# John-Jumper/Upside-MD

Measured on AMD Instinct MI355X. Metric: MD steps/sec (force evals/sec) per 300-res protein, higher is better.
Workload: dtype f32; 1 GPU; syn300_10A: 300-res synthetic protein, full side-chain BP, 10 A pair list (BASELINE.json configs[2]); 4096 independent replicas per GPU, T=0.8, dt=0.009, Langevin thermostat every round; replicas_per_gpu=4096, n_atom=900, settle_steps=100

## Files before the change

upside-md_amd/csrc/kernels_batch_impl.h:

```cpp
#pragma once
template <bool PAIR>
__global__ void __launch_bounds__(1024) PG_KERNEL_ATTR k_batch(BatchArgs A) {
    extern __shared__ __attribute__((aligned(16))) float lds[];
    const int w = blockIdx.x;
    int i = 0;
    while (i + 1 < A.n && w >= A.e[i].wg_end) ++i;
    const BatchEntryHdr& h = A.e[i];
    const int local = w - (i ? A.e[i - 1].wg_end : 0);
    const BX B = {local % h.gx, h.gx, local / h.gx, h.gy};
    const unsigned char* arg = A.blob + h.off;
    if constexpr (!PAIR) {
        const upk_igraph_t& G = *(const upk_igraph_t*)arg;
        const upk_rotamer_t& R = *(const upk_rotamer_t*)arg;
        switch (h.kind) {
            case BK_CHECK: d_pairlist_check(G, B, lds); break;
            case BK_BUILD_ROT: d_pairlist_build<true, UPK_IT_ROTAMER>(G, h.i0, h.i1, B, lds); break;
            case BK_BUILD_COV: d_pairlist_build<true, UPK_IT_HBOND_COVERAGE>(G, h.i0, h.i1, B, lds); break;
            case BK_BUILD_ENV: d_pairlist_build<true, UPK_IT_ENVIRONMENT>(G, h.i0, h.i1, B, lds); break;
            case BK_BUILD_HB: d_pairlist_build<true, UPK_IT_PROTEIN_HBOND>(G, h.i0, h.i1, B, lds); break;
            case BK_REFINE: d_pairlist_refine<false, unsigned short>(G, h.i0, h.i1, B, lds); break;
            case BK_REFINE_SYM: d_pairlist_refine<true, int>(G, h.i0, h.i1, B, lds); break;
            case BK_REFINE_SHORT: d_pairlist_refine_short(G, h.i0, B, lds); break;
            case BK_ORDER: d_pairlist_order(G, h.i0, B, lds); break;
            case BK_CLEAR_SLOTS: d_rotamer_clear_slots(R, B, lds); break;
            case BK_BUILD_SLOTS: d_rotamer_build_slots(R, B, lds); break;
            case BK_NBR_SLOTS: d_rotamer_nbr_slots(R, B, lds); break;
            case BK_SLOTS_BOTH: {
                d_rotamer_build_slots(R, B, lds);
                __syncthreads();
                const BX B1 = {0, 1, B.by, B.gy};
                d_rotamer_nbr_slots(R, B1, lds);
            } break;
            default: break;
        }
    } else {
        const upk_igraph_t& G = *(const upk_igraph_t*)arg;
        const PairArgs& P = *(const PairArgs*)(arg + ((sizeof(upk_igraph_t) + 15) & ~(size_t)15));
        switch (h.kind) {
            case BK_ROWS_HB_FWD: d_pair_rows<UPK_IT_PROTEIN_HBOND, 3, 0, false>(G, P, B, lds); break;
            case BK_ROWS_HB_BWD: d_pair_rows<UPK_IT_PROTEIN_HBOND, 3, 2, false>(G, P, B, lds); break;
            case BK_ROWS_ENV_FWD: d_pair_rows<UPK_IT_ENVIRONMENT, 1, 0, false>(G, P, B, lds); break;
            case BK_COV_ROWS2: d_cov_rows2<2, false>(G, P, B, lds); break;
            case BK_COV_ROWS2_POLY: d_cov_rows2<2, true>(G, P, B, lds); break;
            case BK_ENV_BWD: d_pair_backward<UPK_IT_ENVIRONMENT, 1, false>(G, P, B, lds); break;
            case BK_COV_BWD2: d_cov_backward2<2, false>(G, P, B, lds); break;
            case BK_COV_BWD2_POLY: d_cov_backward2<2, true>(G, P, B, lds); break;
            case BK_BWD_FINISH: d_pair_backward_finish(G, h.i0, h.d0, B, lds); break;
            default: break;
        }
    }
}

extern "C" void* upk_batch_create() { return new BatchState; }
extern "C" void upk_batch_destroy(void* b) {
    BatchState* s = (BatchState*)b;
    if (s && env_set("UPSIDE_HIP_FUSE_STATS")) fprintf(stderr, "merged launches: %ld launches for %ld kernels\n", s->n_merged, s->n_items);
    delete s;
}
extern "C" int upk_batch_begin(const upk_launch_t* L) {
    BatchState* s = batch_of(L);
    if (!s) return 0;
    UPK_FLUSH(L);
    s->open = true; s->chain = 0; s->chains.clear(); s->chain_fused.clear(); s->skip_nbr_slots = false;
    return 0;
}
extern "C" void upk_batch_chain(const upk_launch_t* L, int chain) { BatchState* s = batch_of(L); if (s) s->chain = chain; }
extern "C" int upk_batch_run(const upk_launch_t* L) {
    BatchState* s = batch_of(L);
    if (!s || !s->open) return 0;
    size_t n_stage = 0;
    for (auto& c : s->chains) n_stage = c.size() > n_stage ? c.size() : n_stage;
    for (size_t st = 0; st < n_stage; ++st) {
        for (int pair = 0; pair < 2; ++pair) {
            BatchArgs A; memset(&A, 0, sizeof(A));
            size_t used = 0, lds = 0; int wg = 0;
            auto launch = [&]() {
                if (!A.n) return;
                if (lds < 64) lds = 64;
                if (pair) hipLaunchKernelGGL(k_batch<true>, dim3(wg), dim3(1024), lds, ST(L), A);
                else hipLaunchKernelGGL(k_batch<false>, dim3(wg), dim3(1024), lds, ST(L), A);
                s->n_merged += 1; s->n_items += A.n;
                memset(&A, 0, sizeof(A)); used = 0; lds = 0; wg = 0;
            };
            for (auto& c : s->chains) {
                if (st >= c.size() || (int)bk_is_pair(c[st].kind) != pair) continue;
                const BatchItem& it = c[st];
                const size_t need = (it.args.size() + 15) & ~(size_t)15;
                if (A.n == BATCH_MAX_ENTRIES || used + need > BATCH_BLOB) launch();
                BatchEntryHdr& h = A.e[A.n++];
                h.kind = it.kind; h.gx = it.gx; h.gy = it.gy; h.i0 = it.i0; h.i1 = it.i1; h.d0 = it.d0; h.off = (int)used;
                memcpy(A.blob + used, it.args.data(), it.args.size()); used += need;
                wg += it.gx * it.gy; h.wg_end = wg;
                if (it.lds > lds) lds = it.lds;
            }
            launch();
        }
    }
    s->chains.clear();
    return launch_status();
}
extern "C" int upk_batch_end(const upk_launch_t* L) {
    BatchState* s = batch_of(L);
    if (!s || !s->open) return 0;
    const int r = upk_batch_run(L);
    s->open = false;
    return r;
}
```

upside-md_amd/csrc/kernels_igraph.hip:

```cpp
#include "igraph_device.h"
#include <cstring>

using namespace up;

#define ST(L) ((hipStream_t)(L)->stream)
#define ROWS_PER_BLOCK 4
#define IG_BLOCK (ROWS_PER_BLOCK * UP_WAVE)
#ifndef UPK_LAUNCH_STATUS_DEFINED
#define UPK_LAUNCH_STATUS_DEFINED
static inline int launch_status() { return (int)hipGetLastError(); }
#endif
static inline unsigned rows_grid(int n_rows) { return n_rows > 0 ? (unsigned)((n_rows + ROWS_PER_BLOCK - 1) / ROWS_PER_BLOCK) : 1u; }

#define C_OUT(c, s)  ((c).out  + (size_t)(s) * (c).n_elem * (c).stride)
#define C_SENS(c, s) ((c).sens + (size_t)(s) * (c).n_elem * (c).stride)


__device__ __forceinline__ float quadspline(const upk_igraph_t& G, const float* __restrict__ p, const float* x1, const float* x2,
                                            float* d1, float* d2) {
    const int ka = G.n_knot_angular, k = G.n_knot;
    const float inv_dx = G.inv_dx, inv_dtheta = G.inv_dtheta;
    const f3 displace = mk3(x2[0] - x1[0], x2[1] - x1[1], x2[2] - x1[2]);
    const f3 rvec1 = mk3(x1[3], x1[4], x1[5]), rvec2 = mk3(x2[3], x2[4], x2[5]);
    const float dist2 = mag2(displace), inv_dist = rsqrt_(dist2);
    const float dist_coord = dist2 * (inv_dist * inv_dx);
    const f3 u = inv_dist * displace;
    const float cos1 = dot(rvec1, u), cos2 = -dot(rvec2, u);
    float a1, da1, a2, da2, wide, dwide, narrow, dnarrow;
    deBoor_vd(a1, da1, p, (cos1 + 1.f) * inv_dtheta + 1.f);
    deBoor_vd(a2, da2, p + ka, (cos2 + 1.f) * inv_dtheta + 1.f);
    clamped_deBoor_vd(wide, dwide, p + 2 * ka, dist_coord, k);
    clamped_deBoor_vd(narrow, dnarrow, p + 2 * ka + k, dist_coord, k);
    const float angular_weight = a1 * a2;
    const float radial_deriv = inv_dx * (dwide + angular_weight * dnarrow);
    const float angular_deriv1 = inv_dtheta * da1 * a2 * narrow;
    const float angular_deriv2 = inv_dtheta * a1 * da2 * narrow;
    const f3 rXX = angular_deriv1 * rvec1 - angular_deriv2 * rvec2;
    const f3 deriv_dir = inv_dist * (rXX - dot(u, rXX) * u);
    const f3 dd = radial_deriv * u + deriv_dir;
    d1[0] = -dd.x; d1[1] = -dd.y; d1[2] = -dd.z;
    d1[3] = angular_deriv1 * u.x; d1[4] = angular_deriv1 * u.y; d1[5] = angular_deriv1 * u.z;
    d2[0] = dd.x; d2[1] = dd.y; d2[2] = dd.z;
    d2[3] = -angular_deriv2 * u.x; d2[4] = -angular_deriv2 * u.y; d2[5] = -angular_deriv2 * u.z;
    return wide + angular_weight * narrow;
}

__device__ __forceinline__ float hbond_coverage_edge(const upk_igraph_t& G, const float* __restrict__ p, const float* x1,
                                                     const float* x2, float* d1, float* d2) {
    const float coverage = quadspline(G, p, x1, x2, d1, d2);
    const float one_m = 1.f - x1[6];
    const float prefactor = one_m * one_m;
#pragma unroll
    for (int c = 0; c < 6; ++c) { d1[c] *= prefactor; d2[c] *= prefactor; }
    d1[6] = -coverage * one_m * 2.f;
    return prefactor * coverage;
}

__device__ __forceinline__ float radial_edge(const float* __restrict__ p, const float* x1, const float* x2, float* d1, float* d2) {
    const float inv_dx = p[0];
    const f3 disp = mk3(x1[0] - x2[0], x1[1] - x2[1], x1[2] - x2[2]);
    const float dist2 = mag2(disp), inv_dist = rsqrt_(dist2 + 1e-7f);
    const float dist_coord = dist2 * (inv_dist * inv_dx);
    float v, dv;
    clamped_deBoor_vd(v, dv, p + 1, dist_coord, 16);
    const float k = inv_dist * inv_dx * dv;
    d1[0] = disp.x * k; d1[1] = disp.y * k; d1[2] = disp.z * k;
    d2[0] = -d1[0]; d2[1] = -d1[1]; d2[2] = -d1[2];
    return v;
}

__device__ __forceinline__ float pair_eval(const upk_igraph_t& G, const float* __restrict__ p, const float* x1, const float* x2,
                                           float* d1, float* d2) {
    switch (G.itype) {
        case UPK_IT_RADIAL: case UPK_IT_HBOND_SC_RADIAL: return radial_edge(p, x1, x2, d1, d2);
        case UPK_IT_HBOND_COVERAGE: return hbond_coverage_edge(G, p, x1, x2, d1, d2);
        case UPK_IT_ENVIRONMENT: return environment_edge(p, x1, x2, d1, d2);
        case UPK_IT_PROTEIN_HBOND: return protein_hbond_edge(p, x1, x2, d1, d2);
        default: return quadspline(G, p, x1, x2, d1, d2);
    }
}

__device__ __forceinline__ bool acceptable_id_pair(int itype, int id1, int id2) {
    switch (itype) {
        case UPK_IT_ROTAMER: return ((unsigned)id1 >> 4) != ((unsigned)id2 >> 4);
        case UPK_IT_HBOND_COVERAGE:
        case UPK_IT_RADIAL: case UPK_IT_HBOND_SC_RADIAL:
        case UPK_IT_ENVIRONMENT: return (2 < id1 - id2) || (2 < id2 - id1);
        default: return true;
    }
}

__device__ __forceinline__ void load_elem(float* x, const upk_coord_t& node, int s, int loc, int dim) {
    const float* p = C_OUT(node, s) + (size_t)loc * node.stride;
#pragma unroll
    for (int c = 0; c < 8; ++c) x[c] = (c < dim) ? p[c] : 0.f;
}

__device__ __forceinline__ void d_pairlist_check(const upk_igraph_t& G, const BX B, float* lds_unused) {
    __shared__ int moved;
    __shared__ float top[2][16];
    const int s = B.by;
    if (threadIdx.x == 0) moved = 0;
    __syncthreads();
    const int n_tot = G.symmetric ? G.n1 : G.n1 + G.n2;
    float d1 = 0.f, d2 = 0.f;
    for (int e = threadIdx.x; e < n_tot; e += blockDim.x) {
        const bool side1 = e < G.n1;
        const int i = side1 ? e : e - G.n1;
        const upk_coord_t& node = side1 ? G.node1 : G.node2;
        const float* x = C_OUT(node, s) + (size_t)(side1 ? G.loc1[i] : G.loc2[i]) * node.stride;
        const float* c = (side1 ? G.cache_pos1 + (size_t)s * G.n1 * 4 : G.cache_pos2 + (size_t)s * G.n2 * 4) + (size_t)i * 4;
        const float4 xv = *(const float4*)x, cv = *(const float4*)c;
        const float x0 = xv.x, x1 = xv.y, x2 = xv.z;
        const float dx = x0 - cv.x, dy = x1 - cv.y, dz = x2 - cv.z;
        const float dd = dx * dx + dy * dy + dz * dz;
        d2 = fmaxf(d2, fminf(d1, dd)); d1 = fmaxf(d1, dd);
        ((float4*)(side1 ? G.cur_pos1 + (size_t)s * G.n1 * 4 : G.cur_pos2 + (size_t)s * G.n2 * 4))[i] = make_float4(x0, x1, x2, 0.f);
    }
    {
#pragma unroll
        for (int off = 32; off > 0; off >>= 1) {
            const float o1 = __shfl_xor(d1, off, UP_WAVE), o2 = __shfl_xor(d2, off, UP_WAVE);
            const float n1 = fmaxf(d1, o1), n2 = fmaxf(fminf(d1, o1), fmaxf(d2, o2));
            d1 = n1; d2 = n2;
        }
        if ((threadIdx.x & 63) == 0) { top[0][threadIdx.x >> 6] = d1; top[1][threadIdx.x >> 6] = d2; }
        __syncthreads();
        if (threadIdx.x == 0) {
            float a = 0.f, b = 0.f;
            for (int w = 0; w < (int)(blockDim.x >> 6); ++w) {
                const float o1 = top[0][w], o2 = top[1][w];
                const float n1 = fmaxf(a, o1), n2 = fmaxf(fminf(a, o1), fmaxf(b, o2));
                a = n1; b = n2;
            }
            const float margin = G.cache_cutoff - G.cutoff;
            if (sqrtf(a) + sqrtf(b) > 0.999f * margin) moved = 1;
        }
    }
    __syncthreads();
    if (moved) {
        for (int e = threadIdx.x; e < n_tot; e += blockDim.x) {
            const bool side1 = e < G.n1;
            const int i = side1 ? e : e - G.n1;
            const upk_coord_t& node = side1 ? G.node1 : G.node2;
            const float* x = C_OUT(node, s) + (size_t)(side1 ? G.loc1[i] : G.loc2[i]) * node.stride;
            float4* c = (float4*)(side1 ? G.cache_pos1 + (size_t)s * G.n1 * 4 : G.cache_pos2 + (size_t)s * G.n2 * 4) + i;
            *c = make_float4(x[0], x[1], x[2], __int_as_float(side1 ? G.id1[i] : G.id2[i]));
        }
        if (G.mark_table) {
            uint4* m = (uint4*)(G.mark_table + (size_t)s * G.mark_stride);
            const int n16 = G.mark_stride / 16;
            for (int i = threadIdx.x; i < n16; i += blockDim.x) m[i] = make_uint4(0, 0, 0, 0);
        }
    }
    if (threadIdx.x == 0) {
        G.rebuild_flag[s] = moved;
        int* fl = UPK_FLAG_LIST(G);
        if (moved) fl[1 + atomicAdd(&fl[0], 1)] = s;
        if (s == 0) G.flagged[(size_t)(G.parity ^ 1) * G.flag_stride] = 0;
    }
}
__global__ void k_pairlist_check(upk_igraph_t G)  { d_pairlist_check(G, BX_REAL, nullptr); }
static inline int upkeep_block(int n_system, int large) { return n_system >= 2 * upk_device_cu_count() ? 256 : large; }
extern "C" int upk_pairlist_check(const upk_launch_t* L, const upk_igraph_t* G) {
    if (batch_add(L, BK_CHECK, 1, L->n_system, 0, G, sizeof(*G))) return 0;
    UPK_FLUSH(L);
    const int n_tot = G->symmetric ? G->n1 : G->n1 + G->n2;
    const int threads = upkeep_block(L->n_system, n_tot <= 256 ? 256 : (n_tot <= 512 ? 512 : 1024));
    hipLaunchKernelGGL(k_pairlist_check, dim3(1, L->n_system), dim3(threads), 0, ST(L), *G);
    return launch_status();
}

static inline int plb_rows(int n_system) { return n_system >= upk_device_cu_count() ? 128 : 64; }
template <int IT>
__device__ __forceinline__ bool plb_id_ok(int id_row_side1, int id_other_side2) {
    if (IT == UPK_IT_ROTAMER) return ((unsigned)(id_row_side1 ^ id_other_side2)) > 15u;
    if (IT == UPK_IT_HBOND_COVERAGE || IT == UPK_IT_ENVIRONMENT || IT == UPK_IT_RADIAL || IT == UPK_IT_HBOND_SC_RADIAL) { const int d = id_row_side1 - id_other_side2; return (d > 2) | (d < -2); }
    return true;
}
__device__ __forceinline__ int plb_node_of(const upk_igraph_t& G, int id) {
    const int nr = (id >> 4) & 15;
    return (id >> 8) + ((-(int)(nr == 6) & G.mark_start6) | (-(int)(nr == 3) & G.mark_start3));
}
template <bool STAGED, int IT>
__device__ __forceinline__ void d_pairlist_build(const upk_igraph_t& G, int blocks1, int rows_per_wg, const BX B, float* plb_lds) {
        float4* oth = (float4*)plb_lds;
    constexpr bool SYM = IT == UPK_IT_ROTAMER || IT == UPK_IT_RADIAL;
    constexpr bool UPPER = IT == UPK_IT_ROTAMER;
    const int* fl = UPK_FLAG_LIST(G);
    const int n_flagged = fl[0];
    const int lane = threadIdx.x & 63, wave = __builtin_amdgcn_readfirstlane(threadIdx.x >> 6), n_wave = blockDim.x >> 6;
    const bool side1 = (int)B.bx < blocks1;
    const int rb = side1 ? B.bx : B.bx - blocks1;
    const int n_my = side1 ? G.n1 : G.n2, n_other = side1 ? G.n2 : G.n1;
    const int n_pad = (n_other + 63) & ~63;
    const int cap = side1 ? G.cap1 : G.cap2;
    const float cut2 = G.cache_cutoff * G.cache_cutoff;
    for (int fi = B.by; fi < n_flagged; fi += B.gy) {
        const int s = fl[1 + fi];
        const float4* src = (const float4*)((side1 ? G.cache_pos2 : G.cache_pos1) + (size_t)s * n_other * 4);
        const float4* mine = (const float4*)((side1 ? G.cache_pos1 : G.cache_pos2) + (size_t)s * n_my * 4);
        if (STAGED) {
            __syncthreads();
            for (int j = threadIdx.x; j < n_pad; j += blockDim.x) oth[j] = j < n_other ? src[j] : make_float4(1e18f, 1e18f, 1e18f, 0.f);
            __syncthreads();
        }
        float4 x_next = make_float4(0.f, 0.f, 0.f, 0.f);
        { const int i0 = rb * rows_per_wg + wave; if (wave < rows_per_wg && i0 < n_my) x_next = mine[i0]; }
        for (int r = wave; r < rows_per_wg; r += n_wave) {
            const int i = rb * rows_per_wg + r;
            if (i >= n_my) break;
            const float4 x = x_next;
            { const int in = i + n_wave; if (r + n_wave < rows_per_wg && in < n_my) x_next = mine[in]; }
            const int my_id = __float_as_int(x.w);
            typedef typename list_word<IT>::type W;
            W* nbr = (side1 ? (W*)G.nbr1 + (size_t)s * G.n1 * G.cap1 : (W*)G.nbr2 + (size_t)s * G.n2 * G.cap2) + (size_t)i * cap;
            int count = 0;
            const int my_node = SYM ? plb_node_of(G, my_id) : 0;
            for (int j0 = UPPER ? ((i + 1) & ~63) : 0; j0 < n_pad; j0 += 64) {
                const int j = j0 + lane;
                float4 y;
                if (STAGED) y = oth[j];
                else y = j < n_other ? src[j] : make_float4(1e18f, 1e18f, 1e18f, 0.f);
                const float d2 = dist2_exact(x.x, x.y, x.z, y.x, y.y, y.z);
                const int oid = __float_as_int(y.w);
                bool hit = (d2 < cut2) & (side1 ? plb_id_ok<IT>(my_id, oid) : plb_id_ok<IT>(oid, my_id));
                if (UPPER) hit = hit & (j > i);
                else if (SYM) hit = hit & (j != i);
                const unsigned long long b = __ballot(hit);
                if (!b) continue;
                const int pos = count + __popcll(b & ((1ull << lane) - 1ull));
                if (hit & (pos < cap)) nbr[pos] = (W)j;
                count += __popcll(b);
                if (SYM && G.mark_table) {
                    const bool up = hit & (j > i);
                    const int key = up ? plb_node_of(G, oid) : -1;
                    const int key_prev = __builtin_amdgcn_update_dpp(-1, key, 0x138 , 0xf, 0xf, false);
                    if (up & (key_prev != key)) {
                        unsigned char* mt = G.mark_table + (size_t)s * G.mark_stride;
                        mt[my_node * G.mark_ld + key] = 1; mt[key * G.mark_ld + my_node] = 1;
                    }
                }
            }
            if (lane == 0) {
                (side1 ? G.cnt1 + (size_t)s * G.n1 : G.cnt2 + (size_t)s * G.n2)[i] = count < cap ? count : cap;
                if (count > cap) *G.error_flag = 1;
            }
        }
    }
}
template <bool STAGED, int IT>
__global__ void __launch_bounds__(1024) k_pairlist_build(upk_igraph_t G, int blocks1, int rows_per_wg)  {
    extern __shared__ __attribute__((aligned(16))) float lds_dyn_[];
    d_pairlist_build<STAGED, IT>(G, blocks1, rows_per_wg, BX_REAL, lds_dyn_);
}
template <int IT>
static void plb_launch(const upk_launch_t* L, const upk_igraph_t* G, dim3 grid, size_t lds, bool staged, int blocks1) {
    const int rows = plb_rows(L->n_system);
    if (staged) hipLaunchKernelGGL((k_pairlist_build<true, IT>), grid, dim3(upkeep_block(L->n_system, 1024)), lds, ST(L), *G, blocks1, rows);
    else hipLaunchKernelGGL((k_pairlist_build<false, IT>), grid, dim3(1024), 0, ST(L), *G, blocks1, rows);
}
extern "C" int upk_pairlist_build(const upk_launch_t* L, const upk_igraph_t* G) { return upk_pairlist_build_sides(L, G, 3); }
extern "C" int upk_pairlist_build_sides(const upk_launch_t* L, const upk_igraph_t* G, int sides) {
    if (!list_words_match(G)) return 9010;
    const int rows = plb_rows(L->n_system);
    const int blocks1 = (sides & 1) ? (G->n1 + rows - 1) / rows : 0;
    const int blocks2 = (G->symmetric || !(sides & 2)) ? 0 : (G->n2 + rows - 1) / rows;
    if (blocks1 + blocks2 == 0) return 0;
    const int n_max = G->n1 > G->n2 ? G->n1 : G->n2;
    const size_t lds = (size_t)((n_max + 63) & ~63) * 16;
    const dim3 grid(blocks1 + blocks2, UPK_FLAG_GRID(L->n_system));
    static const bool force_unstaged = env_int("UPSIDE_HIP_PLB_UNSTAGED", 0) != 0;
    const bool staged = lds <= 150 * 1024 && !force_unstaged;
    if (staged) {
        const int bk = G->itype == UPK_IT_ROTAMER ? BK_BUILD_ROT : G->itype == UPK_IT_HBOND_COVERAGE ? BK_BUILD_COV : G->itype == UPK_IT_ENVIRONMENT ? BK_BUILD_ENV
                     : G->itype == UPK_IT_PROTEIN_HBOND ? BK_BUILD_HB : 0;
        if (bk && batch_add(L, bk, (int)grid.x, (int)grid.y, lds, G, sizeof(*G), nullptr, 0, blocks1, rows)) return 0;
    }
    UPK_FLUSH(L);
    switch (G->itype) {
        case UPK_IT_ROTAMER: plb_launch<UPK_IT_ROTAMER>(L, G, grid, lds, staged, blocks1); break;
        case UPK_IT_HBOND_COVERAGE: plb_launch<UPK_IT_HBOND_COVERAGE>(L, G, grid, lds, staged, blocks1); break;
        case UPK_IT_ENVIRONMENT: plb_launch<UPK_IT_ENVIRONMENT>(L, G, grid, lds, staged, blocks1); break;
        case UPK_IT_RADIAL: plb_launch<UPK_IT_RADIAL>(L, G, grid, lds, staged, blocks1); break;
        case UPK_IT_HBOND_SC_RADIAL: plb_launch<UPK_IT_HBOND_SC_RADIAL>(L, G, grid, lds, staged, blocks1); break;
        default: plb_launch<UPK_IT_PROTEIN_HBOND>(L, G, grid, lds, staged, blocks1); break;
    }
    return launch_status();
}

#ifndef PLR_BLOCK
#define PLR_BLOCK 256
#endif
#ifndef PLR_ROWS
#define PLR_ROWS 256
#endif
#ifndef PLR_DEPTH
#define PLR_DEPTH 2
#endif
static_assert(PLR_ROWS <= 64 * (PLR_BLOCK / 64), "a wavefront of the refine keeps the positions and list lengths of its rows one per lane: at most 64 rows per wavefront");
typedef float plr_v2 __attribute__((ext_vector_type(2)));
__device__ __forceinline__ plr_v2 dist2_exact2(plr_v2 ax, plr_v2 ay, plr_v2 az, plr_v2 bx, plr_v2 by, plr_v2 bz) {
#pragma clang fp contract(off)
    const plr_v2 dx = ax - bx, dy = ay - by, dz = az - bz;
    const plr_v2 xx = dx * dx, yy = dy * dy, zz = dz * dz;
    const plr_v2 s = xx + yy;
    return s + zz;
}
template <bool SYM, typename W>
__device__ __forceinline__ void d_pairlist_refine(const upk_igraph_t& G, int side, int rows_per_wg, const BX B, float* plr_lds) {
        float4* oth = (float4*)plr_lds;
    const int s = B.by;
    const int lane = threadIdx.x & 63, wave = __builtin_amdgcn_readfirstlane(threadIdx.x >> 6), n_wave = blockDim.x >> 6;
    const bool rows1 = side == 1;
    const int n_rows = rows1 ? G.n1 : G.n2, n_other = rows1 ? G.n2 : G.n1;
    const int cap = rows1 ? G.cap1 : G.cap2;
    const float4* src = (const float4*)((rows1 ? G.cur_pos2 : G.cur_pos1) + (size_t)s * n_other * 4);
    const float4* mine = (const float4*)((rows1 ? G.cur_pos1 : G.cur_pos2) + (size_t)s * n_rows * 4);
    for (int j = threadIdx.x; j <= n_other; j += blockDim.x) oth[j] = j < n_other ? src[j] : make_float4(1e18f, 1e18f, 1e18f, 0.f);
    __syncthreads();
    const int dead = n_other;
    const W* nbr_base = (const W*)(rows1 ? G.nbr1 : G.nbr2) + (size_t)s * n_rows * cap;
    const int* cnt_arr = (rows1 ? G.cnt1 : G.cnt2) + (size_t)s * n_rows;
    W* hit_base = (W*)(rows1 ? G.hit1 : G.hit2) + (size_t)s * n_rows * cap;
    int* hcnt = (rows1 ? G.hcnt1 : G.hcnt2) + (size_t)s * n_rows;
    int* hlo = (SYM && G.hlo1) ? G.hlo1 + (size_t)s * n_rows : nullptr;
    const float cut2 = G.cutoff * G.cutoff;
    const int jmask = G.nbr_j_bits ? (1 << G.nbr_j_bits) - 1 : 0x7fffffff;
    const int per_wave = (rows_per_wg + n_wave - 1) / n_wave;
    const int r0 = B.bx * rows_per_wg + wave * per_wave;
    int r1 = r0 + per_wave; { const int wg_end = (B.bx + 1) * rows_per_wg; if (r1 > wg_end) r1 = wg_end; if (r1 > n_rows) r1 = n_rows; }
    if (r0 >= r1) return;
    const bool have = r0 + lane < r1;
    const float4 my_x = have ? mine[r0 + lane] : make_float4(0.f, 0.f, 0.f, 0.f);
    const int my_cnt = have ? cnt_arr[r0 + lane] : 0;
    int my_n = 0, my_lo = 0;
    auto bcast = [&](float v, int l) { return __int_as_float(__builtin_amdgcn_readlane(__float_as_int(v), l)); };
    auto fetch_pair = [&](int ra, int& a, int& b) {
        a = dead; b = dead;
        if (ra < r1) {
            const int la = ra - r0;
            const int cA = __builtin_amdgcn_readlane(my_cnt, la & 63), cB = ra + 1 < r1 ? __builtin_amdgcn_readlane(my_cnt, (la + 1) & 63) : 0;
            if (lane < cA) a = nbr_base[(size_t)ra * cap + lane];
            if (lane < cB) b = nbr_base[(size_t)(ra + 1) * cap + lane];
        }
    };
    int qA[PLR_DEPTH], qB[PLR_DEPTH];
#pragma unroll
    for (int d = 0; d < PLR_DEPTH; ++d) fetch_pair(r0 + 2 * d, qA[d], qB[d]);
    for (int ra = r0; ra < r1; ra += 2) {
        const int la = ra - r0, lb = la + 1;
        const bool hasB = ra + 1 < r1;
        const int cntA = __builtin_amdgcn_readlane(my_cnt, la), cntB = hasB ? __builtin_amdgcn_readlane(my_cnt, lb & 63) : 0;
        int wA = qA[0], wB = qB[0];
#pragma unroll
        for (int d = 0; d + 1 < PLR_DEPTH; ++d) { qA[d] = qA[d + 1]; qB[d] = qB[d + 1]; }
        fetch_pair(ra + 2 * PLR_DEPTH, qA[PLR_DEPTH - 1], qB[PLR_DEPTH - 1]);
        plr_v2 xx, xy, xz;
        xx.x = bcast(my_x.x, la); xy.x = bcast(my_x.y, la); xz.x = bcast(my_x.z, la);
        xx.y = bcast(my_x.x, lb & 63); xy.y = bcast(my_x.y, lb & 63); xz.y = bcast(my_x.z, lb & 63);
        const W* nbrA = nbr_base + (size_t)ra * cap; const W* nbrB = nbrA + cap;
        W* outA = hit_base + (size_t)ra * cap; W* outB = outA + cap;
        int na = 0, nb = 0, loa = 0, lob = 0;
        const int cmax = cntA > cntB ? cntA : cntB;
        for (int k0 = 0; k0 < cmax; k0 += 64) {
            const int k = k0 + lane;
            if (k0) { wA = k < cntA ? nbrA[k] : dead; wB = k < cntB ? nbrB[k] : dead; }
            const int jA = wA & jmask, jB = wB & jmask;
            const float4 yA = oth[jA], yB = oth[jB];
            plr_v2 yx, yy, yz; yx.x = yA.x; yx.y = yB.x; yy.x = yA.y; yy.y = yB.y; yz.x = yA.z; yz.y = yB.z;
            const plr_v2 d2 = dist2_exact2(xx, xy, xz, yx, yy, yz);
            const bool hitA = d2.x < cut2, hitB = d2.y < cut2;
            const unsigned long long mA = __builtin_amdgcn_ballot_w64(hitA), mB = __builtin_amdgcn_ballot_w64(hitB);
            const unsigned long long below = (1ull << lane) - 1ull;
            if (hitA) outA[na + __popcll(mA & below)] = (W)wA;
            if (hitB) outB[nb + __popcll(mB & below)] = (W)wB;
            na += __popcll(mA); nb += __popcll(mB);
            if (SYM) { loa += __popcll(__builtin_amdgcn_ballot_w64(hitA && jA < ra)); lob += __popcll(__builtin_amdgcn_ballot_w64(hitB && jB < ra + 1)); }
        }
        if (lane == la) { my_n = na; my_lo = loa; }
        if (hasB && lane == lb) { my_n = nb; my_lo = lob; }
    }
    if (have) { hcnt[r0 + lane] = my_n; if (SYM && hlo) hlo[r0 + lane] = my_lo; }
}
template <bool SYM, typename W>
__global__ void __launch_bounds__(PLR_BLOCK) k_pairlist_refine(upk_igraph_t G, int side, int rows_per_wg)  {
    extern __shared__ __attribute__((aligned(16))) float lds_dyn_[];
    d_pairlist_refine<SYM, W>(G, side, rows_per_wg, BX_REAL, lds_dyn_);
}
__device__ __forceinline__ void d_pairlist_refine_short(const upk_igraph_t& G, int side, const BX B, float* lds_unused) {
    const int s = B.by, row = B.bx * blockDim.x + threadIdx.x;
    const bool rows1 = side == 1;
    const int n_rows = rows1 ? G.n1 : G.n2, n_other = rows1 ? G.n2 : G.n1;
    if (row >= n_rows) return;
    const int cap = rows1 ? G.cap1 : G.cap2;
    const float4* src = (const float4*)((rows1 ? G.cur_pos2 : G.cur_pos1) + (size_t)s * n_other * 4);
    const float4 x = ((const float4*)((rows1 ? G.cur_pos1 : G.cur_pos2) + (size_t)s * n_rows * 4))[row];
    typedef list_word<UPK_IT_PROTEIN_HBOND>::type W;
    const W* nbr = (const W*)(rows1 ? G.nbr1 : G.nbr2) + ((size_t)s * n_rows + row) * cap;
    W* hit = (W*)(rows1 ? G.hit1 : G.hit2) + ((size_t)s * n_rows + row) * cap;
    const int cnt = ((rows1 ? G.cnt1 : G.cnt2) + (size_t)s * n_rows)[row];
    const float cut2 = G.cutoff * G.cutoff;
    const int jmask = G.nbr_j_bits ? (1 << G.nbr_j_bits) - 1 : 0x7fffffff;
    int n = 0;
    for (int k0 = 0; k0 < cnt; k0 += 4) {
        int w[4]; float4 y[4];
#pragma unroll
        for (int u = 0; u < 4; ++u) w[u] = nbr[k0 + u < cnt ? k0 + u : k0];
#pragma unroll
        for (int u = 0; u < 4; ++u) y[u] = src[w[u] & jmask];
#pragma unroll
        for (int u = 0; u < 4; ++u)
            if (k0 + u < cnt && dist2_exact(x.x, x.y, x.z, y[u].x, y[u].y, y[u].z) < cut2) hit[n++] = (W)w[u];
    }
    ((rows1 ? G.hcnt1 : G.hcnt2) + (size_t)s * n_rows)[row] = n;
}
__global__ void __launch_bounds__(256) k_pairlist_refine_short(upk_igraph_t G, int side)  { d_pairlist_refine_short(G, side, BX_REAL, nullptr); }
extern "C" int upk_pairlist_refine(const upk_launch_t* L, const upk_igraph_t* G, int side) {
    const bool rows1 = side == 1;
    const int n_rows = rows1 ? G->n1 : G->n2, n_other = rows1 ? G->n2 : G->n1;
    if (n_rows < 1) return 0;
    if (G->itype == UPK_IT_PROTEIN_HBOND && !G->symmetric) {
        if (batch_add(L, BK_REFINE_SHORT, (n_rows + 1023) / 1024, L->n_system, 0, G, sizeof(*G), nullptr, 0, side)) return 0;
        UPK_FLUSH(L);
        hipLaunchKernelGGL(k_pairlist_refine_short, dim3((n_rows + 255) / 256, L->n_system), dim3(256), 0, ST(L), *G, side);
        return launch_status();
    }
    if (!list_words_match(G)) return 9010;
    if ((G->symmetric != 0) == (G->word16 != 0)) return 9011;
    const size_t lds = (size_t)((n_other > 0 ? n_other : 0) + 1) * 16;
    if (lds > 150 * 1024) return 9006;
    int rows_per_wg = L->n_system >= upk_device_cu_count() ? PLR_ROWS : (L->n_system >= 16 ? 64 : 16);
    {
        if (n_rows <= 512 && rows_per_wg > 128) rows_per_wg = 128;
    }
    {
        const int rows_b = rows_per_wg * 4;
        if (batch_add(L, G->symmetric ? BK_REFINE_SYM : BK_REFINE, (n_rows + rows_b - 1) / rows_b, L->n_system, lds, G, sizeof(*G), nullptr, 0, side, rows_b)) return 0;
    }
    UPK_FLUSH(L);
    const dim3 grid((n_rows + rows_per_wg - 1) / rows_per_wg, L->n_system);
    if (G->symmetric) hipLaunchKernelGGL((k_pairlist_refine<true, int>), grid, dim3(PLR_BLOCK), lds, ST(L), *G, side, rows_per_wg);
    else hipLaunchKernelGGL((k_pairlist_refine<false, unsigned short>), grid, dim3(PLR_BLOCK), lds, ST(L), *G, side, rows_per_wg);

    return launch_status();
}

#define PLO_BINS 1024
template <typename KeyFn>
__device__ __forceinline__ void order_rows(unsigned short* __restrict__ ord, int n_rows, KeyFn key, int* hist, int* scratch) {
    hist[threadIdx.x] = 0;
    __syncthreads();
    for (int r = threadIdx.x; r < n_rows; r += blockDim.x) atomicAdd(&hist[PLO_BINS - 1 - key(r)], 1);
    __syncthreads();
    const int lane = threadIdx.x & 63, wave = threadIdx.x >> 6;
    const int v = hist[threadIdx.x];
    int incl = v;
#pragma unroll
    for (int off = 1; off < 64; off <<= 1) { const int t = __shfl_up(incl, off, UP_WAVE); if (lane >= off) incl += t; }
    if (lane == 63) scratch[wave] = incl;
    __syncthreads();
    if (threadIdx.x == 0) { int acc = 0; for (int w = 0; w < (int)(blockDim.x >> 6); ++w) { const int t = scratch[w]; scratch[w] = acc; acc += t; } }
    __syncthreads();
    hist[threadIdx.x] = scratch[wave] + incl - v;
    __syncthreads();
    for (int r = threadIdx.x; r < n_rows; r += blockDim.x) ord[atomicAdd(&hist[PLO_BINS - 1 - key(r)], 1)] = (unsigned short)r;
    __syncthreads();
}
__device__ __forceinline__ void d_pairlist_order(const upk_igraph_t& G, int side, const BX B, float* lds_unused) {
    __shared__ int hist[PLO_BINS], scratch[16];
    const int s = B.bx;
    const bool rows1 = side == 1;
    const int n_rows = rows1 ? G.n1 : G.n2;
    const int* hcnt = (rows1 ? G.hcnt1 : G.hcnt2) + (size_t)s * n_rows;
    order_rows((rows1 ? G.ord1 : G.ord2) + (size_t)s * n_rows, n_rows,
               [&](int r) { const int c = hcnt[r]; return c < PLO_BINS ? c : PLO_BINS - 1; }, hist, scratch);
    if (G.symmetric && G.hlo1) {
        const int* hlo = G.hlo1 + (size_t)s * n_rows;
        order_rows(G.ord1u + (size_t)s * n_rows, n_rows,
                   [&](int r) { const int c = hcnt[r] - hlo[r]; return c < PLO_BINS ? c : PLO_BINS - 1; }, hist, scratch);
    }
}
__global__ void __launch_bounds__(PLO_BINS) k_pairlist_order(upk_igraph_t G, int side)  { d_pairlist_order(G, side, BX_REAL, nullptr); }
extern "C" int upk_pairlist_order(const upk_launch_t* L, const upk_igraph_t* G, int side) {
    const int n_rows = side == 1 ? G->n1 : G->n2;
    if (n_rows < 1) return 0;
    if (n_rows > 65535) return 9009;
    if (batch_add(L, BK_ORDER, L->n_system, 1, 0, G, sizeof(*G), nullptr, 0, side)) return 0;
    UPK_FLUSH(L);
    hipLaunchKernelGGL(k_pairlist_order, dim3(L->n_system), dim3(PLO_BINS), 0, ST(L), *G, side);
    return launch_status();
}

__global__ void k_igraph_rowsum(upk_igraph_t G, int side, float* __restrict__ out, long out_sys_stride, int out_stride, int out_comp,
                                int out_row0, float* __restrict__ own_grad) {
    const int s = blockIdx.y;
    const int lane = threadIdx.x & 63;
    const int n_rows = side == 1 ? G.n1 : G.n2;
    const float cut2 = G.cutoff * G.cutoff;
    for (int row = blockIdx.x * ROWS_PER_BLOCK + (threadIdx.x >> 6); row < n_rows; row += gridDim.x * ROWS_PER_BLOCK) {
        const int cap = side == 1 ? G.cap1 : G.cap2;
        const int* lists = side == 1 ? G.nbr1 : G.nbr2;
        const size_t row_at = ((size_t)s * n_rows + row) * cap;
        const int cnt = (side == 1 ? G.cnt1 + (size_t)s * G.n1 : G.cnt2 + (size_t)s * G.n2)[row];
        float xr[8];
        if (side == 1) load_elem(xr, G.node1, s, G.loc1[row], G.dim1); else load_elem(xr, G.node2, s, G.loc2[row], G.dim2);
        const int tr = side == 1 ? G.type1[row] : G.type2[row];
        float acc = 0.f, og[8];
#pragma unroll
        for (int c = 0; c < 8; ++c) og[c] = 0.f;
        for (int k = lane; k < cnt; k += 64) {
            const int j = list_word_at(lists, row_at + k, G.word16);
            float xo[8], d1[8], d2[8];
#pragma unroll
            for (int c = 0; c < 8; ++c) { d1[c] = 0.f; d2[c] = 0.f; }
            if (side == 1) load_elem(xo, G.node2, s, G.loc2[j], G.dim2); else load_elem(xo, G.node1, s, G.loc1[j], G.dim1);
            if (!(dist2_exact(xr[0], xr[1], xr[2], xo[0], xo[1], xo[2]) < cut2)) continue;
            const int t1 = side == 1 ? tr : G.type1[j], t2 = side == 1 ? G.type2[j] : tr;
            const float* p = G.param + (size_t)(t1 * G.n_type2 + t2) * G.n_param;
            acc += side == 1 ? pair_eval(G, p, xr, xo, d1, d2) : pair_eval(G, p, xo, xr, d1, d2);
#pragma unroll
            for (int c = 0; c < 8; ++c) og[c] += side == 1 ? d1[c] : d2[c];
        }
        acc = wave_sum(acc);
        if (lane == 0) out[(size_t)s * out_sys_stride + (size_t)(out_row0 + row) * out_stride + out_comp] = acc;
        if (own_grad) {
#pragma unroll
            for (int c = 0; c < 8; ++c) og[c] = wave_sum(og[c]);
            if (lane == 0) {
                float* o = own_grad + ((size_t)s * n_rows + row) * 8;
#pragma unroll
                for (int c = 0; c < 8; ++c) o[c] = og[c];
            }
        }
    }
}
extern "C" int upk_igraph_rowsum(const upk_launch_t* L, const upk_igraph_t* G, int side, float* out, long out_sys_stride,
                                 int out_stride, int out_comp, int out_row0, float* own_grad) {
    UPK_FLUSH(L);
    const int n_rows = side == 1 ? G->n1 : G->n2;
    hipLaunchKernelGGL(k_igraph_rowsum, dim3(rows_grid(n_rows), L->n_system), dim3(IG_BLOCK), 0, ST(L), *G, side,
                       out, out_sys_stride, out_stride, out_comp, out_row0, own_grad);
    return launch_status();
}

__global__ void k_igraph_grad(upk_igraph_t G, int side, int sens_mode, const float* __restrict__ sens1, const float* __restrict__ sens2,
                              long sens_sys_stride, int sens_stride) {
    const int s = blockIdx.y;
    const int lane = threadIdx.x & 63;
    const int n_rows = side == 1 ? G.n1 : G.n2;
    const int dim_row = side == 1 ? G.dim1 : G.dim2;
    const float cut2 = G.cutoff * G.cutoff;
    const float* S1 = sens1 ? sens1 + (size_t)s * sens_sys_stride : nullptr;
    const float* S2 = sens2 ? sens2 + (size_t)s * sens_sys_stride : nullptr;
    for (int row = blockIdx.x * ROWS_PER_BLOCK + (threadIdx.x >> 6); row < n_rows; row += gridDim.x * ROWS_PER_BLOCK) {
        const int cap = side == 1 ? G.cap1 : G.cap2;
        const int* lists = side == 1 ? G.nbr1 : G.nbr2;
        const size_t row_at = ((size_t)s * n_rows + row) * cap;
        const int cnt = (side == 1 ? G.cnt1 + (size_t)s * G.n1 : G.cnt2 + (size_t)s * G.n2)[row];
        float xr[8];
        if (side == 1) load_elem(xr, G.node1, s, G.loc1[row], G.dim1); else load_elem(xr, G.node2, s, G.loc2[row], G.dim2);
        const int tr = side == 1 ? G.type1[row] : G.type2[row];
        float srow = 0.f;
        if (sens_mode == 1 && side == 1) srow = S1[(size_t)row * sens_stride];
        if (sens_mode == 2 && side == 2) srow = S2[(size_t)row * sens_stride];
        if (sens_mode == 3) srow = side == 1 ? S1[(size_t)row * sens_stride] : S2[(size_t)row * sens_stride];
        float acc[8];
#pragma unroll
        for (int c = 0; c < 8; ++c) acc[c] = 0.f;
        for (int k = lane; k < cnt; k += 64) {
            const int j = list_word_at(lists, row_at + k, G.word16);
            float xo[8], d1[8], d2[8];
#pragma unroll
            for (int c = 0; c < 8; ++c) { d1[c] = 0.f; d2[c] = 0.f; }
            if (side == 1) load_elem(xo, G.node2, s, G.loc2[j], G.dim2); else load_elem(xo, G.node1, s, G.loc1[j], G.dim1);
            if (!(dist2_exact(xr[0], xr[1], xr[2], xo[0], xo[1], xo[2]) < cut2)) continue;
            const int t1 = side == 1 ? tr : G.type1[j], t2 = side == 1 ? G.type2[j] : tr;
            const float* p = G.param + (size_t)(t1 * G.n_type2 + t2) * G.n_param;
            if (side == 1) pair_eval(G, p, xr, xo, d1, d2); else pair_eval(G, p, xo, xr, d1, d2);
            float ps;
            if (sens_mode == 0) ps = 1.f;
            else if (sens_mode == 1) ps = side == 1 ? srow : S1[(size_t)j * sens_stride];
            else if (sens_mode == 2) ps = side == 2 ? srow : S2[(size_t)j * sens_stride];
            else ps = srow + (side == 1 ? S2[(size_t)j * sens_stride] : S1[(size_t)j * sens_stride]);
            const float* dr = side == 1 ? d1 : d2;
#pragma unroll
            for (int c = 0; c < 8; ++c) acc[c] += ps * dr[c];
        }
#pragma unroll
// ... 164 lines not shown
```

Before: 221,900 system-steps/s.

## Cull pair-list build candidates with per-run bounding spheres before exact distance tests

In the staged pair-list build, each wavefront now takes a run of up to 8 rows and computes a bounding-box center and radius for them. It then filters all other-side positions in LDS against that sphere widened by the cutoff, writing the survivors into a per-wave LDS index buffer. The exact per-row distance and ballot tests then run only over the survivors, which is meant to cut the all-pairs work when pair lists are rebuilt. In exchange it uses extra LDS and adds filtering overhead, and it only helps when rebuilds are a meaningful share of step time.

```diff
diff --git a/upside-md_amd/csrc/kernels_batch_impl.h b/upside-md_amd/csrc/kernels_batch_impl.h
--- a/upside-md_amd/csrc/kernels_batch_impl.h
+++ b/upside-md_amd/csrc/kernels_batch_impl.h
@@ -14,10 +14,10 @@
         const upk_rotamer_t& R = *(const upk_rotamer_t*)arg;
         switch (h.kind) {
             case BK_CHECK: d_pairlist_check(G, B, lds); break;
-            case BK_BUILD_ROT: d_pairlist_build<true, UPK_IT_ROTAMER>(G, h.i0, h.i1, B, lds); break;
-            case BK_BUILD_COV: d_pairlist_build<true, UPK_IT_HBOND_COVERAGE>(G, h.i0, h.i1, B, lds); break;
-            case BK_BUILD_ENV: d_pairlist_build<true, UPK_IT_ENVIRONMENT>(G, h.i0, h.i1, B, lds); break;
-            case BK_BUILD_HB: d_pairlist_build<true, UPK_IT_PROTEIN_HBOND>(G, h.i0, h.i1, B, lds); break;
+            case BK_BUILD_ROT: d_pairlist_build<true, UPK_IT_ROTAMER>(G, h.i0, h.i1, h.d0 != 0., B, lds); break;
+            case BK_BUILD_COV: d_pairlist_build<true, UPK_IT_HBOND_COVERAGE>(G, h.i0, h.i1, h.d0 != 0., B, lds); break;
+            case BK_BUILD_ENV: d_pairlist_build<true, UPK_IT_ENVIRONMENT>(G, h.i0, h.i1, h.d0 != 0., B, lds); break;
+            case BK_BUILD_HB: d_pairlist_build<true, UPK_IT_PROTEIN_HBOND>(G, h.i0, h.i1, h.d0 != 0., B, lds); break;
             case BK_REFINE: d_pairlist_refine<false, unsigned short>(G, h.i0, h.i1, B, lds); break;
             case BK_REFINE_SYM: d_pairlist_refine<true, int>(G, h.i0, h.i1, B, lds); break;
             case BK_REFINE_SHORT: d_pairlist_refine_short(G, h.i0, B, lds); break;
diff --git a/upside-md_amd/csrc/kernels_igraph.hip b/upside-md_amd/csrc/kernels_igraph.hip
--- a/upside-md_amd/csrc/kernels_igraph.hip
+++ b/upside-md_amd/csrc/kernels_igraph.hip
@@ -1,4 +1,5 @@
 #include "igraph_device.h"
+#include "plb_cull.h"
 #include <cstring>
 
 using namespace up;
@@ -182,11 +183,38 @@
     const int nr = (id >> 4) & 15;
     return (id >> 8) + ((-(int)(nr == 6) & G.mark_start6) | (-(int)(nr == 3) & G.mark_start3));
 }
+template <int IT>
+__device__ __forceinline__ void plb_trip(const upk_igraph_t& G, int s, bool side1, int i, const float4 x, int my_id, int my_node, int j, const float4 y,
+                                         float cut2, typename list_word<IT>::type* nbr, int cap, int lane, int& count) {
+    constexpr bool SYM = IT == UPK_IT_ROTAMER || IT == UPK_IT_RADIAL;
+    constexpr bool UPPER = IT == UPK_IT_ROTAMER;
+    typedef typename list_word<IT>::type W;
+    const float d2 = dist2_exact(x.x, x.y, x.z, y.x, y.y, y.z);
+    const int oid = __float_as_int(y.w);
+    bool hit = (d2 < cut2) & (side1 ? plb_id_ok<IT>(my_id, oid) : plb_id_ok<IT>(oid, my_id));
+    if (UPPER) hit = hit & (j > i);
+    else if (SYM) hit = hit & (j != i);
+    const unsigned long long b = __ballot(hit);
+    if (!b) return;
+    const int pos = count + __popcll(b & ((1ull << lane) - 1ull));
+    if (hit & (pos < cap)) nbr[pos] = (W)j;
+    count += __popcll(b);
+    if (SYM && G.mark_table) {
+        const bool up = hit & (j > i);
+        const int key = up ? plb_node_of(G, oid) : -1;
+        const int key_prev = __builtin_amdgcn_update_dpp(-1, key, 0x138 , 0xf, 0xf, false);
+        if (up & (key_prev != key)) {
+            unsigned char* mt = G.mark_table + (size_t)s * G.mark_stride;
+            mt[my_node * G.mark_ld + key] = 1; mt[key * G.mark_ld + my_node] = 1;
+        }
+    }
+}
 template <bool STAGED, int IT>
-__device__ __forceinline__ void d_pairlist_build(const upk_igraph_t& G, int blocks1, int rows_per_wg, const BX B, float* plb_lds) {
+__device__ __forceinline__ void d_pairlist_build(const upk_igraph_t& G, int blocks1, int rows_per_wg, bool cull, const BX B, float* plb_lds) {
         float4* oth = (float4*)plb_lds;
     constexpr bool SYM = IT == UPK_IT_ROTAMER || IT == UPK_IT_RADIAL;
     constexpr bool UPPER = IT == UPK_IT_ROTAMER;
+    typedef typename list_word<IT>::type W;
     const int* fl = UPK_FLAG_LIST(G);
     const int n_flagged = fl[0];
     const int lane = threadIdx.x & 63, wave = __builtin_amdgcn_readfirstlane(threadIdx.x >> 6), n_wave = blockDim.x >> 6;
@@ -200,10 +228,69 @@
         const int s = fl[1 + fi];
         const float4* src = (const float4*)((side1 ? G.cache_pos2 : G.cache_pos1) + (size_t)s * n_other * 4);
         const float4* mine = (const float4*)((side1 ? G.cache_pos1 : G.cache_pos2) + (size_t)s * n_my * 4);
+        W* nbr_s = side1 ? (W*)G.nbr1 + (size_t)s * G.n1 * G.cap1 : (W*)G.nbr2 + (size_t)s * G.n2 * G.cap2;
+        int* cnt_s = side1 ? G.cnt1 + (size_t)s * G.n1 : G.cnt2 + (size_t)s * G.n2;
         if (STAGED) {
             __syncthreads();
-            for (int j = threadIdx.x; j < n_pad; j += blockDim.x) oth[j] = j < n_other ? src[j] : make_float4(1e18f, 1e18f, 1e18f, 0.f);
+            for (int j = threadIdx.x; j < n_pad + (cull ? 1 : 0); j += blockDim.x) oth[j] = j < n_other ? src[j] : make_float4(1e18f, 1e18f, 1e18f, 0.f);
             __syncthreads();
+        }
+        if (STAGED && cull) {
+            const int row0 = rb * rows_per_wg;
+            const int row_end = min(row0 + rows_per_wg, n_my);
+            const int run = min(PLB_RUN, max(1, rows_per_wg / n_wave));
+            unsigned short* buf = (unsigned short*)(oth + n_pad + 1) + (size_t)wave * plb_cull_buf_len(n_pad);
+            auto bcast = [&](float v, int l) { return __int_as_float(__builtin_amdgcn_readlane(__float_as_int(v), l)); };
+            float4 x_next = make_float4(0.f, 0.f, 0.f, 0.f);
+            { const int i0 = row0 + wave * run; if (i0 < row_end) x_next = mine[min(i0 + min(lane, run - 1), row_end - 1)]; }
+            for (int i0 = row0 + wave * run; i0 < row_end; i0 += n_wave * run) {
+                const int n_r = min(run, row_end - i0);
+                const float4 xr = x_next;
+                { const int in = i0 + n_wave * run; if (in < row_end) x_next = mine[min(in + min(lane, run - 1), row_end - 1)]; }
+                float lox = bcast(xr.x, 0), loy = bcast(xr.y, 0), loz = bcast(xr.z, 0), hix = lox, hiy = loy, hiz = loz;
+                for (int k = 1; k < n_r; ++k) {
+                    const float ax = bcast(xr.x, k), ay = bcast(xr.y, k), az = bcast(xr.z, k);
+                    lox = fminf(lox, ax); loy = fminf(loy, ay); loz = fminf(loz, az);
+                    hix = fmaxf(hix, ax); hiy = fmaxf(hiy, ay); hiz = fmaxf(hiz, az);
+                }
+                const float cx = 0.5f * (lox + hix), cy = 0.5f * (loy + hiy), cz = 0.5f * (loz + hiz);
+                const float r2_lane = plb_dist2(xr.x, xr.y, xr.z, cx, cy, cz);
+                float r2 = 0.f;
+                for (int k = 0; k < n_r; ++k) r2 = fmaxf(r2, bcast(r2_lane, k));
+                const float reach2 = plb_cull_reach2(G.cache_cutoff, r2);
+                int n_surv = 0;
+                for (int j0 = UPPER ? ((i0 + 1) & ~63) : 0; j0 < n_pad; j0 += 64) {
+                    const int j = j0 + lane;
+                    const float4 y = oth[j];
+                    const bool keep = plb_dist2(y.x, y.y, y.z, cx, cy, cz) < reach2;
+                    const unsigned long long b = __ballot(keep);
+                    if (!b) continue;
+                    if (keep) buf[n_surv + __popcll(b & ((1ull << lane) - 1ull))] = (unsigned short)j;
+                    n_surv += __popcll(b);
+                }
+                buf[n_surv + lane] = (unsigned short)n_pad;
+                __builtin_amdgcn_fence(__ATOMIC_RELEASE, "wavefront"); __builtin_amdgcn_wave_barrier(); __builtin_amdgcn_fence(__ATOMIC_ACQUIRE, "wavefront");
+                for (int k = 0; k < n_r; ++k) {
+                    const int i = i0 + k;
+                    const float4 x = make_float4(bcast(xr.x, k), bcast(xr.y, k), bcast(xr.z, k), bcast(xr.w, k));
+                    const int my_id = __float_as_int(x.w);
+                    const int my_node = SYM ? plb_node_of(G, my_id) : 0;
+                    W* nbr = nbr_s + (size_t)i * cap;
+                    int count = 0;
+                    int j_next = buf[lane];
+                    for (int t0 = 0; t0 < n_surv; t0 += 64) {
+                        const int j = j_next;
+                        if (t0 + 64 < n_surv) j_next = buf[t0 + 64 + lane];
+                        plb_trip<IT>(G, s, side1, i, x, my_id, my_node, j, oth[j], cut2, nbr, cap, lane, count);
+                    }
+                    if (lane == 0) {
+                        cnt_s[i] = count < cap ? count : cap;
+                        if (count > cap) *G.error_flag = 1;
+                    }
+                }
+                __builtin_amdgcn_fence(__ATOMIC_RELEASE, "wavefront"); __builtin_amdgcn_wave_barrier(); __builtin_amdgcn_fence(__ATOMIC_ACQUIRE, "wavefront");
+            }
+            continue;
         }
         float4 x_next = make_float4(0.f, 0.f, 0.f, 0.f);
         { const int i0 = rb * rows_per_wg + wave; if (wave < rows_per_wg && i0 < n_my) x_next = mine[i0]; }
@@ -213,8 +300,7 @@
             const float4 x = x_next;
             { const int in = i + n_wave; if (r + n_wave < rows_per_wg && in < n_my) x_next = mine[in]; }
             const int my_id = __float_as_int(x.w);
-            typedef typename list_word<IT>::type W;
-            W* nbr = (side1 ? (W*)G.nbr1 + (size_t)s * G.n1 * G.cap1 : (W*)G.nbr2 + (size_t)s * G.n2 * G.cap2) + (size_t)i * cap;
+            W* nbr = nbr_s + (size_t)i * cap;
             int count = 0;
             const int my_node = SYM ? plb_node_of(G, my_id) : 0;
             for (int j0 = UPPER ? ((i + 1) & ~63) : 0; j0 < n_pad; j0 += 64) {
@@ -222,43 +308,25 @@
                 float4 y;
                 if (STAGED) y = oth[j];
                 else y = j < n_other ? src[j] : make_float4(1e18f, 1e18f, 1e18f, 0.f);
-                const float d2 = dist2_exact(x.x, x.y, x.z, y.x, y.y, y.z);
-                const int oid = __float_as_int(y.w);
-                bool hit = (d2 < cut2) & (side1 ? plb_id_ok<IT>(my_id, oid) : plb_id_ok<IT>(oid, my_id));
-                if (UPPER) hit = hit & (j > i);
-                else if (SYM) hit = hit & (j != i);
-                const unsigned long long b = __ballot(hit);
-                if (!b) continue;
-                const int pos = count + __popcll(b & ((1ull << lane) - 1ull));
-                if (hit & (pos < cap)) nbr[pos] = (W)j;
-                count += __popcll(b);
-                if (SYM && G.mark_table) {
-                    const bool up = hit & (j > i);
-                    const int key = up ? plb_node_of(G, oid) : -1;
-                    const int key_prev = __builtin_amdgcn_update_dpp(-1, key, 0x138 , 0xf, 0xf, false);
-                    if (up & (key_prev != key)) {
-                        unsigned char* mt = G.mark_table + (size_t)s * G.mark_stride;
-                        mt[my_node * G.mark_ld + key] = 1; mt[key * G.mark_ld + my_node] = 1;
-                    }
-                }
+                plb_trip<IT>(G, s, side1, i, x, my_id, my_node, j, y, cut2, nbr, cap, lane, count);
             }
             if (lane == 0) {
-                (side1 ? G.cnt1 + (size_t)s * G.n1 : G.cnt2 + (size_t)s * G.n2)[i] = count < cap ? count : cap;
+                cnt_s[i] = count < cap ? count : cap;
                 if (count > cap) *G.error_flag = 1;
             }
         }
     }
 }
 template <bool STAGED, int IT>
-__global__ void __launch_bounds__(1024) k_pairlist_build(upk_igraph_t G, int blocks1, int rows_per_wg)  {
+__global__ void __launch_bounds__(1024) k_pairlist_build(upk_igraph_t G, int blocks1, int rows_per_wg, int cull)  {
     extern __shared__ __attribute__((aligned(16))) float lds_dyn_[];
-    d_pairlist_build<STAGED, IT>(G, blocks1, rows_per_wg, BX_REAL, lds_dyn_);
+    d_pairlist_build<STAGED, IT>(G, blocks1, rows_per_wg, cull != 0, BX_REAL, lds_dyn_);
 }
 template <int IT>
-static void plb_launch(const upk_launch_t* L, const upk_igraph_t* G, dim3 grid, size_t lds, bool staged, int blocks1) {
+static void plb_launch(const upk_launch_t* L, const upk_igraph_t* G, dim3 grid, size_t lds, bool staged, int blocks1, int cull) {
     const int rows = plb_rows(L->n_system);
-    if (staged) hipLaunchKernelGGL((k_pairlist_build<true, IT>), grid, dim3(upkeep_block(L->n_system, 1024)), lds, ST(L), *G, blocks1, rows);
-    else hipLaunchKernelGGL((k_pairlist_build<false, IT>), grid, dim3(1024), 0, ST(L), *G, blocks1, rows);
+    if (staged) hipLaunchKernelGGL((k_pairlist_build<true, IT>), grid, dim3(upkeep_block(L->n_system, 1024)), lds, ST(L), *G, blocks1, rows, cull);
+    else hipLaunchKernelGGL((k_pairlist_build<false, IT>), grid, dim3(1024), 0, ST(L), *G, blocks1, rows, 0);
 }
 extern "C" int upk_pairlist_build(const upk_launch_t* L, const upk_igraph_t* G) { return upk_pairlist_build_sides(L, G, 3); }
 extern "C" int upk_pairlist_build_sides(const upk_launch_t* L, const upk_igraph_t* G, int sides) {
@@ -268,23 +336,29 @@
     const int blocks2 = (G->symmetric || !(sides & 2)) ? 0 : (G->n2 + rows - 1) / rows;
     if (blocks1 + blocks2 == 0) return 0;
     const int n_max = G->n1 > G->n2 ? G->n1 : G->n2;
-    const size_t lds = (size_t)((n_max + 63) & ~63) * 16;
+    const int n_pad_max = (n_max + 63) & ~63;
+    size_t lds = (size_t)n_pad_max * 16;
     const dim3 grid(blocks1 + blocks2, UPK_FLAG_GRID(L->n_system));
     static const bool force_unstaged = env_int("UPSIDE_HIP_PLB_UNSTAGED", 0) != 0;
     const bool staged = lds <= 150 * 1024 && !force_unstaged;
+    static const bool cull_on = env_int("UPSIDE_HIP_PLB_CULL", 1) != 0;
+    const bool in_batch = batch_of(L) && batch_of(L)->open;
+    const size_t lds_cull = plb_cull_lds_bytes(n_pad_max, (in_batch ? 1024 : upkeep_block(L->n_system, 1024)) / 64);
+    const int cull = staged && cull_on && n_pad_max > PLB_CULL_MIN_PAD && lds_cull <= 150 * 1024;
+    if (cull) lds = lds_cull;
     if (staged) {
         const int bk = G->itype == UPK_IT_ROTAMER ? BK_BUILD_ROT : G->itype == UPK_IT_HBOND_COVERAGE ? BK_BUILD_COV : G->itype == UPK_IT_ENVIRONMENT ? BK_BUILD_ENV
                      : G->itype == UPK_IT_PROTEIN_HBOND ? BK_BUILD_HB : 0;
-        if (bk && batch_add(L, bk, (int)grid.x, (int)grid.y, lds, G, sizeof(*G), nullptr, 0, blocks1, rows)) return 0;
+        if (bk && batch_add(L, bk, (int)grid.x, (int)grid.y, lds, G, sizeof(*G), nullptr, 0, blocks1, rows, (double)cull)) return 0;
     }
     UPK_FLUSH(L);
     switch (G->itype) {
-        case UPK_IT_ROTAMER: plb_launch<UPK_IT_ROTAMER>(L, G, grid, lds, staged, blocks1); break;
-        case UPK_IT_HBOND_COVERAGE: plb_launch<UPK_IT_HBOND_COVERAGE>(L, G, grid, lds, staged, blocks1); break;
-        case UPK_IT_ENVIRONMENT: plb_launch<UPK_IT_ENVIRONMENT>(L, G, grid, lds, staged, blocks1); break;
-        case UPK_IT_RADIAL: plb_launch<UPK_IT_RADIAL>(L, G, grid, lds, staged, blocks1); break;
-        case UPK_IT_HBOND_SC_RADIAL: plb_launch<UPK_IT_HBOND_SC_RADIAL>(L, G, grid, lds, staged, blocks1); break;
-        default: plb_launch<UPK_IT_PROTEIN_HBOND>(L, G, grid, lds, staged, blocks1); break;
+        case UPK_IT_ROTAMER: plb_launch<UPK_IT_ROTAMER>(L, G, grid, lds, staged, blocks1, cull); break;
+        case UPK_IT_HBOND_COVERAGE: plb_launch<UPK_IT_HBOND_COVERAGE>(L, G, grid, lds, staged, blocks1, cull); break;
+        case UPK_IT_ENVIRONMENT: plb_launch<UPK_IT_ENVIRONMENT>(L, G, grid, lds, staged, blocks1, cull); break;
+        case UPK_IT_RADIAL: plb_launch<UPK_IT_RADIAL>(L, G, grid, lds, staged, blocks1, cull); break;
+        case UPK_IT_HBOND_SC_RADIAL: plb_launch<UPK_IT_HBOND_SC_RADIAL>(L, G, grid, lds, staged, blocks1, cull); break;
+        default: plb_launch<UPK_IT_PROTEIN_HBOND>(L, G, grid, lds, staged, blocks1, cull); break;
     }
     return launch_status();
 }
diff --git a/upside-md_amd/csrc/plb_cull.h b/upside-md_amd/csrc/plb_cull.h
--- /dev/null
+++ b/upside-md_amd/csrc/plb_cull.h
@@ -0,0 +1,34 @@
+#pragma once
+#include <math.h>
+
+#if defined(__HIPCC__)
+#define PLB_HD __host__ __device__ __forceinline__
+#else
+#define PLB_HD static inline
+#endif
+
+#ifndef PLB_RUN
+#define PLB_RUN 8
+#endif
+#define PLB_CULL_EPS 1.52587890625e-05f
+#define PLB_CULL_MIN_PAD 128
+
+PLB_HD float plb_dist2(float ax, float ay, float az, float bx, float by, float bz) {
+#if defined(__HIP_DEVICE_COMPILE__)
+    const float dx = __fsub_rn(ax, bx), dy = __fsub_rn(ay, by), dz = __fsub_rn(az, bz);
+    return __fadd_rn(__fadd_rn(__fmul_rn(dx, dx), __fmul_rn(dy, dy)), __fmul_rn(dz, dz));
+#else
+    volatile float dx = ax - bx, dy = ay - by, dz = az - bz;
+    volatile float xx = dx * dx, yy = dy * dy, zz = dz * dz;
+    volatile float s = xx + yy;
+    return s + zz;
+#endif
+}
+
+PLB_HD float plb_cull_reach2(float cache_cutoff, float r2_run) {
+    const float reach = cache_cutoff + sqrtf(r2_run);
+    return (reach * reach) * (1.f + PLB_CULL_EPS);
+}
+
+PLB_HD int plb_cull_buf_len(int n_pad) { return n_pad + 64; }
+PLB_HD size_t plb_cull_lds_bytes(int n_pad, int n_wave) { return (size_t)(n_pad + 1) * 16 + (size_t)n_wave * plb_cull_buf_len(n_pad) * 2; }
```

Result: no change. 221,200 system-steps/s (-0.3%).
